# duanyiqun/DiffusionDepth

Measured on NVIDIA H100. Metric: depth maps/sec @ KITTI 352x1216, Swin-L, 20 DDIM steps, higher is better.
Workload: dtype f32 (fp32-grade products on wgmma: 3-pass fp16 split, fp32 accumulate)

## Files before the change

### diffusiondepth_b200/_cabi.py

```python
import ctypes as C
import os

_HERE = os.path.dirname(os.path.abspath(__file__))
_LIB = None


class EngineError(RuntimeError):
    """Raised for any non-zero status coming back across the C ABI."""


class DDConfig(C.Structure):
    _fields_ = [("abi_version", C.c_int32), ("variant", C.c_int32), ("batch", C.c_int32),
                ("latent_h", C.c_int32), ("latent_w", C.c_int32), ("cond_h", C.c_int32),
                ("cond_w", C.c_int32), ("num_inference_steps", C.c_int32), ("device", C.c_int32),
                ("flags", C.c_int32)]


class DDProducerConfig(C.Structure):
    _fields_ = [("num_levels", C.c_int32), ("channels", C.c_int32 * 4), ("heights", C.c_int32 * 4),
                ("widths", C.c_int32 * 4), ("has_neck", C.c_int32)]


class DDBackboneConfig(C.Structure):
    _fields_ = [("kind", C.c_int32), ("embed_dims", C.c_int32), ("depths", C.c_int32 * 4),
# ... 42 lines not shown
    "dd_denoiser_backward": (C.c_int, [C.c_void_p, C.c_void_p, C.c_void_p, C.POINTER(C.c_int64), C.c_void_p,
                                       C.c_void_p, C.c_void_p, C.POINTER(C.c_void_p), C.c_void_p, C.c_size_t,
                                       C.c_void_p]),
    "dd_denoiser_relu_inputs": (C.c_int, [C.c_void_p, C.c_void_p, C.c_void_p, C.POINTER(C.c_int64),
                                          C.POINTER(C.c_void_p), C.c_void_p, C.c_size_t, C.c_void_p]),
    "dd_denoise_backward": (C.c_int, [C.c_void_p, C.c_void_p, C.c_void_p, C.c_void_p, C.c_void_p, C.c_void_p,
                                      C.c_void_p, C.POINTER(C.c_void_p), C.POINTER(C.c_void_p), C.c_void_p,
                                      C.c_void_p, C.c_size_t, C.c_void_p]),
    "dd_decode": (C.c_int, [C.c_void_p, C.c_void_p, C.c_void_p, C.c_void_p, C.c_void_p, C.c_size_t, C.c_void_p]),
    "dd_decode_backward": (C.c_int, [C.c_void_p, C.c_void_p, C.c_void_p, C.c_void_p, C.POINTER(C.c_void_p),
                                     C.c_void_p, C.c_size_t, C.c_void_p]),
    "dd_encode": (C.c_int, [C.c_void_p, C.c_void_p, C.c_int32, C.c_int32, C.c_void_p, C.c_void_p]),
    "dd_set_codec_mode": (C.c_int, [C.c_void_p, C.c_int32]),
    "dd_codec_batch_stats": (C.c_int, [C.c_void_p, C.c_void_p, C.c_int32, C.POINTER(C.c_int32), C.c_void_p]),
    "dd_set_producer_mode": (C.c_int, [C.c_void_p, C.c_int32]),
    "dd_producer_batch_stats": (C.c_int, [C.c_void_p, C.c_void_p, C.c_int64, C.POINTER(C.c_int32), C.c_void_p]),
    "dd_producer_bn_info": (C.c_int, [C.c_void_p, C.c_int32, C.c_char_p, C.c_int32, C.POINTER(C.c_int32),
                                      C.POINTER(C.c_int64), C.POINTER(C.c_int32)]),
    "dd_last_launch_count": (C.c_int64, [C.c_void_p]),
    "dd_poll_status": (C.c_int, [C.c_void_p, C.c_void_p]),
    "dd_conv3x3": (C.c_int, [C.c_void_p, C.c_void_p, C.c_void_p, C.c_void_p, C.c_void_p, C.c_int32, C.c_int32,
                             C.c_int32, C.c_int32, C.c_int32, C.c_void_p, C.c_size_t, C.c_void_p]),
    "dd_conv3x3_workspace_bytes": (C.c_size_t, [C.c_int32, C.c_int32, C.c_int32, C.c_int32, C.c_int32]),
    "dd_conv3x3_wgrad": (C.c_int, [C.c_void_p, C.c_void_p, C.c_void_p, C.c_void_p, C.c_void_p, C.c_int32, C.c_int32,
                                   C.c_int32, C.c_int32, C.c_int32, C.c_void_p, C.c_size_t, C.c_void_p]),
    "dd_conv3x3_wgrad_workspace_bytes": (C.c_size_t, [C.c_int32, C.c_int32, C.c_int32, C.c_int32, C.c_int32]),
    "dd_gen_layer": (C.c_int, [C.c_void_p, C.POINTER(DDGenLayerDesc), C.c_void_p, C.c_void_p, C.c_void_p, C.c_void_p,
                               C.POINTER(C.c_void_p), C.c_void_p, C.c_void_p, C.c_void_p, C.c_void_p,
                               C.POINTER(C.c_int32), C.c_void_p]),
    "dd_window_attention": (C.c_int, [C.c_void_p, C.c_void_p, C.c_void_p, C.c_void_p, C.c_void_p, C.c_int32,
                                      C.c_int32, C.c_int32, C.c_int32, C.c_int32, C.c_int32, C.POINTER(C.c_int32),
                                      C.c_void_p]),
    "dd_factor_attention": (C.c_int, [C.c_void_p, C.c_void_p, C.POINTER(C.c_void_p), C.POINTER(C.c_void_p), C.c_void_p,
                                      C.c_int32, C.c_int32, C.c_int32, C.c_int32, C.POINTER(C.c_int32), C.c_void_p]),
    "dd_depthwise_conv": (C.c_int, [C.c_void_p, C.c_void_p, C.c_void_p, C.c_void_p, C.POINTER(C.c_void_p), C.c_void_p,
                                    C.c_void_p, C.c_void_p, C.c_int32, C.c_int32, C.c_int32, C.c_int32, C.c_int32,
                                    C.c_int32, C.c_int32, C.POINTER(C.c_int32), C.c_void_p]),
    "dd_layer_norm": (C.c_int, [C.c_void_p, C.c_void_p, C.c_void_p, C.c_void_p, C.c_void_p, C.c_int32, C.c_int32,
                                C.c_float, C.c_void_p]),
    "dd_bench_gemm": (C.c_int, [C.c_void_p, C.c_int32, C.c_int32, C.c_int32, C.c_int32, C.c_int32, C.POINTER(C.c_float)]),
    "dd_bench_conv": (C.c_int, [C.c_void_p, C.c_int32, C.c_int32, C.c_int32, C.POINTER(C.c_float), C.c_void_p,
                                C.c_size_t, C.c_void_p]),
    "dd_bench_pred_fold": (C.c_int, [C.c_void_p, C.c_int32, C.POINTER(C.c_float), C.c_void_p, C.c_size_t,
                                     C.c_void_p]),
}

# ... 32 lines not shown
```

### diffusiondepth_b200/csrc/conv_halo.cuh

```cuda
#pragma once
#include "conv_common.cuh"

namespace dd {

constexpr int HALO_TH = 16;
constexpr int HALO_TW = 8;

template <int CIN, int COUT, int BK>
struct HaloCfg {
  static_assert(BK == 16 || BK == 32, "bad K chunk");
  static_assert((CIN % BK == 0 || CIN < BK) && CIN % 16 == 0, "bad K chunk");
  static constexpr int KC = (CIN + BK - 1) / BK;
  static constexpr int KSTEPS = (CIN < BK ? CIN : BK) / 16;
  static constexpr int ROW_BYTES = BK * 2;
  static constexpr int STRIP_ROWS = (HALO_TH + 2) * HALO_TW;
  static constexpr int STRIP_BYTES = STRIP_ROWS * ROW_BYTES;
  static constexpr int STRIP_PAD = (STRIP_BYTES + 1023) / 1024 * 1024;
  static constexpr int DX_STRIDE = 2 * STRIP_PAD;
  static constexpr int A_SLOT = 3 * DX_STRIDE;
  static constexpr int A_SLOTS = 2;
  static constexpr int B_TILE = COUT * ROW_BYTES;
  static constexpr int B_TILE_PAD = (B_TILE + 1023) / 1024 * 1024;
  static constexpr int B_SLOT = 2 * B_TILE_PAD;
  static constexpr int NWG = COUT > 128 ? 2 : 1;
  static constexpr int NW = COUT / NWG;
  static constexpr int THREADS = 128 * (1 + NWG);
  static constexpr int CH = NWG > 1 ? 16 : (NW < 32 ? NW : 32);
  static constexpr int LD = CH + 1;
  static constexpr int STAGE_BYTES = NWG * 128 * LD * 4;
  static constexpr int CTRL_BYTES = 1024;
  static constexpr int BUDGET = 227 * 1024 - 1024 - CTRL_BYTES - STAGE_BYTES - A_SLOTS * A_SLOT;
  static constexpr int B_SLOTS_RAW = BUDGET / B_SLOT;
  static constexpr bool B_RESIDENT = (9 * KC * B_SLOT <= 40 * 1024) && (9 * KC <= B_SLOTS_RAW);
  static constexpr int B_SLOTS = B_RESIDENT ? 9 * KC : (B_SLOTS_RAW > 8 ? 8 : B_SLOTS_RAW);
  static_assert(B_SLOTS >= 2, "B ring too small");
  static_assert(NWG == 1 || B_SLOTS >= 3, "256-wide layers: the producer must be able to run two taps ahead");
  static constexpr int SMEM_BYTES = A_SLOTS * A_SLOT + B_SLOTS * B_SLOT + 1024 + CTRL_BYTES + STAGE_BYTES;
  static_assert(SMEM_BYTES <= 232448, "exceeds the 227 KB dynamic shared memory limit");
  static constexpr int A_TX = 6 * STRIP_BYTES;
  static constexpr int B_TX = 2 * B_TILE;
  static constexpr int GROUP_CH = COUT / 4;
  static constexpr int GPW = NW >= GROUP_CH ? NW / GROUP_CH : 1;
  static_assert(NW % GROUP_CH == 0, "a warpgroup's columns cover whole GroupNorm groups");
};

template <int CIN, int COUT, int BK, int EPI>
__global__ void __launch_bounds__((HaloCfg<CIN, COUT, BK>::THREADS), 1)
conv3x3_halo_kernel(const __grid_constant__ CUtensorMap tmA_hi, const __grid_constant__ CUtensorMap tmA_lo,
                    const __grid_constant__ CUtensorMap tmB_hi, const __grid_constant__ CUtensorMap tmB_lo,
                    const ConvArgs p) {
  using C = HaloCfg<CIN, COUT, BK>;
  constexpr int NW = C::NW;
  extern __shared__ uint8_t smem_raw[];
  uint8_t* smem = reinterpret_cast<uint8_t*>((reinterpret_cast<uintptr_t>(smem_raw) + 1023) & ~uintptr_t(1023));
  uint8_t* a_ring = smem;
  uint8_t* b_ring = smem + C::A_SLOTS * C::A_SLOT;
  uint8_t* ctrl = b_ring + C::B_SLOTS * C::B_SLOT;
  uint64_t* a_full = reinterpret_cast<uint64_t*>(ctrl);
  uint64_t* a_empty = a_full + C::A_SLOTS;
  uint64_t* b_full = a_empty + C::A_SLOTS;
  uint64_t* b_empty = b_full + C::B_SLOTS;
  float* red = reinterpret_cast<float*>(b_empty + C::B_SLOTS);
  float* stage = reinterpret_cast<float*>(ctrl + C::CTRL_BYTES);

  const int warp = threadIdx.x >> 5;
  const int lane = threadIdx.x & 31;

  if (threadIdx.x == 0) {
    tma_prefetch_desc(&tmA_hi);
    tma_prefetch_desc(&tmA_lo);
    tma_prefetch_desc(&tmB_hi);
    tma_prefetch_desc(&tmB_lo);
    for (int s = 0; s < C::A_SLOTS; ++s) {
      mbar_init(&a_full[s], 1);
      mbar_init(&a_empty[s], C::NWG);
    }
    for (int s = 0; s < C::B_SLOTS; ++s) {
      mbar_init(&b_full[s], 1);
      mbar_init(&b_empty[s], C::NWG);
    }
    fence_barrier_init();
  }
  __syncthreads();

  if (warp < 4) {
    if constexpr (C::NWG > 1) setmaxnreg_dec<40>();
    if (warp == 0) {
      const bool leader = elect_one();
      int sa = 0;
      uint32_t pa = 0;
      for (int tile = blockIdx.x; tile < p.num_tiles; tile += gridDim.x) {
        const int tx = tile % p.tiles_x, ty = (tile / p.tiles_x) % p.tiles_y, img = tile / (p.tiles_x * p.tiles_y);
        const int x0 = tx * HALO_TW, y0 = ty * HALO_TH;
        for (int kc = 0; kc < C::KC; ++kc) {
          mbar_wait(&a_empty[sa], pa ^ 1);
          uint8_t* s = a_ring + sa * C::A_SLOT;
          if (leader) {
            mbar_arrive_expect_tx(&a_full[sa], C::A_TX);
#pragma unroll
            for (int dx = 0; dx < 3; ++dx) {
              tma_load_4d(s + (2 * dx) * C::STRIP_PAD, &tmA_hi, &a_full[sa], kc * BK, x0 + dx - 1, y0 - 1, img);
              tma_load_4d(s + (2 * dx + 1) * C::STRIP_PAD, &tmA_lo, &a_full[sa], kc * BK, x0 + dx - 1, y0 - 1, img);
            }
          }
          __syncwarp();
          if (++sa == C::A_SLOTS) {
            sa = 0;
            pa ^= 1;
          }
        }
      }
    } else if (warp == 1) {
      const bool leader = elect_one();
      int sb = 0;
      uint32_t pb = 0;
      for (int tile = blockIdx.x; tile < p.num_tiles; tile += gridDim.x) {
        if (C::B_RESIDENT && tile != static_cast<int>(blockIdx.x)) break;
        for (int kc = 0; kc < C::KC; ++kc) {
          for (int tap = 0; tap < 9; ++tap) {
            mbar_wait(&b_empty[sb], pb ^ 1);
            uint8_t* s = b_ring + sb * C::B_SLOT;
            if (leader) {
              mbar_arrive_expect_tx(&b_full[sb], C::B_TX);
              tma_load_3d(s, &tmB_hi, &b_full[sb], kc * BK, 0, tap);
              tma_load_3d(s + C::B_TILE_PAD, &tmB_lo, &b_full[sb], kc * BK, 0, tap);
            }
            __syncwarp();
            if (++sb == C::B_SLOTS) {
              sb = 0;
              pb ^= 1;
            }
          }
        }
      }
    }
  } else {
    if constexpr (C::NWG > 1) setmaxnreg_inc<232>();
    const int wg = (warp >> 2) - 1;
    const int t = threadIdx.x & 127;
    const int q = t >> 5;
    const bool signal = (t == 0);
    float* S = stage + wg * 128 * C::LD;
    const int m = t;
    const int r = m >> 3, c = m & 7;
    const uint32_t b_off = static_cast<uint32_t>(wg * NW);
    int sa = 0, sb = 0, par = 0;
    uint32_t pa = 0, pb = 0;
    float acc[2][NW / 2];

    for (int tile = blockIdx.x; tile < p.num_tiles; tile += gridDim.x) {
      int prev_b = -1, prev_a = -1;
      auto retire_prev = [&]() {
        mbar_arrive_if(&b_empty[prev_b < 0 ? 0 : prev_b], signal && prev_b >= 0);
        mbar_arrive_if(&a_empty[prev_a < 0 ? 0 : prev_a], signal && prev_a >= 0);
        prev_b = prev_a = -1;
      };
      {
        for (int kc = 0; kc < C::KC; ++kc) {
          mbar_wait(&a_full[sa], pa);
          const uint32_t a_base = smem_u32(a_ring + sa * C::A_SLOT);
          for (int tap = 0; tap < 9; ++tap) {
            const int dy = tap / 3, dx = tap % 3;
            mbar_wait(&b_full[sb], C::B_RESIDENT ? 0u : pb);
            const uint32_t sa_hi = a_base + dx * C::DX_STRIDE + dy * HALO_TW * C::ROW_BYTES;
            const uint32_t sa_lo = sa_hi + C::STRIP_PAD;
            const uint32_t sb_hi = smem_u32(b_ring + sb * C::B_SLOT) + b_off * C::ROW_BYTES;
            const uint32_t sb_lo = sb_hi + C::B_TILE_PAD;
            wgmma_fence();
#pragma unroll
            for (int h = 0; h < 2; ++h) {
              const uint32_t ho = static_cast<uint32_t>(h * 64 * C::ROW_BYTES);
#pragma unroll
              for (int k = 0; k < C::KSTEPS; ++k) {
                const uint64_t a_hi = wgmma_desc(sa_hi + ho + k * 32, C::ROW_BYTES);
                const uint64_t a_lo = wgmma_desc(sa_lo + ho + k * 32, C::ROW_BYTES);
                const uint64_t b_hi = wgmma_desc(sb_hi + k * 32, C::ROW_BYTES);
                const uint64_t b_lo = wgmma_desc(sb_lo + k * 32, C::ROW_BYTES);
                wgmma_f16<NW>(acc[h], a_lo, b_hi, (kc | tap | k) != 0 ? 1u : 0u);
                wgmma_f16<NW>(acc[h], a_hi, b_lo, 1u);
                wgmma_f16<NW>(acc[h], a_hi, b_hi, 1u);
              }
            }
            wgmma_commit();
            wgmma_wait<1>();
            retire_prev();
            if (!C::B_RESIDENT) prev_b = sb;
            if (tap == 8) prev_a = sa;
            if (++sb == C::B_SLOTS) {
              sb = 0;
              pb ^= 1;
            }
          }
          if (++sa == C::A_SLOTS) {
            sa = 0;
            pa ^= 1;
          }
        }
      }
      wgmma_wait<0>();
      wgmma_fence_regs(acc[0]);
      wgmma_fence_regs(acc[1]);
      retire_prev();

      const int tx = tile % p.tiles_x, ty = (tile / p.tiles_x) % p.tiles_y, img = tile / (p.tiles_x * p.tiles_y);
      const int x = tx * HALO_TW + c, y = ty * HALO_TH + r;
      const bool valid = (x < p.W) && (y < p.H);
      const size_t pix = (static_cast<size_t>(img) * p.H + y) * p.W + x;
      const uint32_t vmask = __ballot_sync(0xffffffffu, valid);
      const uint32_t row_off = static_cast<uint32_t>(pix * COUT);
      float tsum[C::GPW], tsq[C::GPW];
#pragma unroll
      for (int g = 0; g < C::GPW; ++g) tsum[g] = tsq[g] = 0.f;
      bool overflow = false;
#pragma unroll
      for (int cj = 0; cj < NW / C::CH; ++cj) {
        const int ch0 = wg * NW + cj * C::CH;
        named_bar_sync(2 + wg, 128);
        stage_acc_cols<NW, C::CH, C::LD>(acc[0], S, 0, cj * C::CH / 8);
        stage_acc_cols<NW, C::CH, C::LD>(acc[1], S, 64, cj * C::CH / 8);
        named_bar_sync(2 + wg, 128);
        float v[C::CH];
#pragma unroll
        for (int j = 0; j < C::CH; ++j) v[j] = fmaf(S[m * C::LD + j], p.acc_scale, __ldg(p.bias + ch0 + j));
        if constexpr (EPI == EPI_F32_STATS) {
          if (valid) {
#pragma unroll
            for (int j = 0; j < C::CH; ++j) {
              const int g = (cj * C::CH + j) / C::GROUP_CH;
              tsum[g] += v[j];
              tsq[g] = fmaf(v[j], v[j], tsq[g]);
            }
          }
        }
        if constexpr (EPI == EPI_F32_STATS || EPI == EPI_F32) {
#pragma unroll
          for (int j = 0; j < C::CH; ++j) S[m * C::LD + j] = v[j];
          __syncwarp();
          if constexpr (C::CH == 32) {
#pragma unroll 8
// ... 14 lines not shown
        } else if (valid) {
          {
            __align__(16) __half hi[C::CH];
            __align__(16) __half lo[C::CH];
#pragma unroll
            for (int j = 0; j < C::CH; ++j) {
              const float s = v[j] * p.split_scale;
              overflow |= (fabsf(s) > 60000.f);
              hi[j] = __float2half_rn(s);
              lo[j] = __float2half_rn(s - __half2float(hi[j]));
            }
            uint4* dh = reinterpret_cast<uint4*>(p.out_hi + pix * COUT + ch0);
            uint4* dl = reinterpret_cast<uint4*>(p.out_lo + pix * COUT + ch0);
#pragma unroll
            for (int j = 0; j < C::CH / 8; ++j) {
              dh[j] = reinterpret_cast<const uint4*>(hi)[j];
              dl[j] = reinterpret_cast<const uint4*>(lo)[j];
            }
          }
        }
      }

      if constexpr (EPI == EPI_F32_STATS) {
        const int cw = wg * 4 + q;
#pragma unroll
        for (int g = 0; g < 4; ++g) {
          const int gl = g - (C::NWG > 1 ? wg * C::GPW : 0);
          float s = 0.f, s2 = 0.f;
#pragma unroll
          for (int k = 0; k < C::GPW; ++k)
            if (k == gl) {
              s = tsum[k];
              s2 = tsq[k];
            }
#pragma unroll
          for (int o = 16; o > 0; o >>= 1) {
            s += __shfl_xor_sync(0xffffffffu, s, o);
            s2 += __shfl_xor_sync(0xffffffffu, s2, o);
          }
          if (lane == 0) {
            red[((par * 4 * C::NWG + cw) * 4 + g) * 2 + 0] = s;
            red[((par * 4 * C::NWG + cw) * 4 + g) * 2 + 1] = s2;
          }
        }
        named_bar_sync(1, 128 * C::NWG);
        const int e = threadIdx.x - 128;
        if (e < 8) {
          const int g = e >> 1, which = e & 1;
          float tt = 0.f;
#pragma unroll
          for (int w = 0; w < 4 * C::NWG; ++w) tt += red[((par * 4 * C::NWG + w) * 4 + g) * 2 + which];
          p.stats_partial[(static_cast<size_t>(tile) * 4 + g) * 2 + which] = tt;
        }
        par ^= 1;
      }
      if constexpr (EPI == EPI_SPLIT) {
        if (overflow) atomicOr(p.status, 1);
      }
    }
  }
}

}
```

### diffusiondepth_b200/csrc/engine.cu

```cuda
#include <cuda.h>
#include <cuda_runtime.h>
#include <math.h>
#include <stdio.h>
#include <stdlib.h>
#include <string.h>

#include <algorithm>
#include <map>
#include <string>
#include <vector>

#include "../../include/dd_engine.h"
#include "kernels.cuh"
#include "convgen.cuh"
#include "conv_halo.cuh"
#include "pred_fold.cuh"
#include "swin.cuh"
#include "mpvit.cuh"
#include "backward.cuh"
#include "codec_train.cuh"
#include "producer_train.cuh"

namespace {

// ... 1074 lines not shown

int dev_alloc(std::vector<void*>& owned, void** p, size_t bytes) {
  cudaError_t err = cudaMalloc(p, bytes);
  if (err != cudaSuccess) return fail(DD_ERR_CUDA, std::string("cudaMalloc: ") + cudaGetErrorString(err));
  owned.push_back(*p);
  return DD_OK;
}
int dev_alloc(dd_engine* e, void** p, size_t bytes) { return dev_alloc(e->owned, p, bytes); }

template <typename T>
int dev_array(dd_engine* e, T** p, size_t elems) {
  return dev_alloc(e->owned, reinterpret_cast<void**>(p), elems * sizeof(T));
}

int alloc_layer(dd_engine* e, ConvLayer& L, int cout, int cin) {
  L.sid = shape_id(cin, cout);
  if (L.sid < 0) return fail(DD_ERR_UNSUPPORTED, "unsupported conv shape");
  const size_t n = static_cast<size_t>(cout) * cin * 9;
  int rc;
  if ((rc = dev_array(e, &L.w_hi, n))) return rc;
  if ((rc = dev_array(e, &L.w_lo, n))) return rc;
  if ((rc = dev_array(e, &L.w_simt, n))) return rc;
  if ((rc = dev_array(e, &L.bias, cout))) return rc;
  if ((rc = make_weight_map(&L.mh_hi, L.w_hi, cout, cin, 9, kHaloBK[L.sid], cout))) return rc;
  return make_weight_map(&L.mh_lo, L.w_lo, cout, cin, 9, kHaloBK[L.sid], cout);
}

constexpr float kProdScale = 16.f;

void bn_fold_host(const float* const* bn, int ch, float* scale, float* shift) {
  for (int c = 0; c < ch; ++c) {
    const double sc = static_cast<double>(bn[0][c]) / sqrt(static_cast<double>(bn[3][c]) + 1e-5);
    scale[c] = static_cast<float>(sc);
    shift[c] = static_cast<float>(static_cast<double>(bn[1][c]) - static_cast<double>(bn[2][c]) * sc);
  }
}
int bn_fold(const float* const* bn, int ch, std::vector<float>& scale, std::vector<float>& shift, cudaStream_t st) {
  std::vector<float> v[4];
  for (int i = 0; i < 4; ++i) {
    v[i].resize(ch);
    CUDA_TRY(cudaMemcpyAsync(v[i].data(), bn[i], ch * 4, cudaMemcpyDeviceToHost, st));
  }
  CUDA_TRY(cudaStreamSynchronize(st));
  scale.resize(ch);
  shift.resize(ch);
  const float* host[4] = {v[0].data(), v[1].data(), v[2].data(), v[3].data()};
  bn_fold_host(host, ch, scale.data(), shift.data());
  return DD_OK;
// ... 2137 lines not shown
  a.H = height;
  a.W = width;
  a.h = h->cfg.latent_h;
  a.w = h->cfg.latent_w;
  dim3 grid((a.w + 15) / 16, (a.h + 15) / 16, h->cfg.batch);
  dd::encoder_kernel<<<grid, 256, 0, st>>>(a);
  return check_launch("encoder");
}

int64_t dd_last_launch_count(dd_handle h) { return h ? h->launches : 0; }

int dd_poll_status(dd_handle h, void* cuda_stream) {
  if (!h) return fail(DD_ERR_INVALID, "null handle");
  if (!h->status) return DD_OK;
  CUDA_TRY(cudaSetDevice(h->cfg.device));
  return poll_status(h, static_cast<cudaStream_t>(cuda_stream));
}

size_t dd_conv3x3_workspace_bytes(int32_t batch, int32_t cin, int32_t cout, int32_t height, int32_t width) {
  Conv3x3Ws v;
  return conv3x3_layout(nullptr, batch, cin, cout, height, width, v);
}

int dd_conv3x3(dd_handle h, const float* x, const float* w, const float* b, float* y, int32_t batch, int32_t cin,
               int32_t cout, int32_t height, int32_t width, void* workspace, size_t workspace_bytes, void* cuda_stream) {
  if (!h || !x || !w || !b || !y) return fail(DD_ERR_INVALID, "null argument");
  const int sid = shape_id(cin, cout);
  if (sid < 0) return fail(DD_ERR_UNSUPPORTED, "conv shape not on the DiffusionDepth hot path");
  if (workspace_bytes < dd_conv3x3_workspace_bytes(batch, cin, cout, height, width) ||
      (reinterpret_cast<uintptr_t>(workspace) & 1023))
    return fail(DD_ERR_INVALID, "conv workspace too small or misaligned");
  cudaStream_t st = static_cast<cudaStream_t>(cuda_stream);
  CUDA_TRY(cudaSetDevice(h->cfg.device));
  const size_t BP = static_cast<size_t>(batch) * height * width;
  const size_t nw = static_cast<size_t>(cin) * cout * 9;
  Conv3x3Ws v;
  conv3x3_layout(workspace, batch, cin, cout, height, width, v);
  CUDA_TRY(cudaMemsetAsync(v.status, 0, 64, st));
  int rc;
  if ((rc = transpose_in(x, v.xn, batch, cin, height * width, st))) return rc;
  float* amax_dev = reinterpret_cast<float*>(v.status) + 8;
  float sx, sw;
  if ((rc = split_scale_of(v.xn, std::min<size_t>(BP * cin, 1u << 30), amax_dev, st, &sx))) return rc;
  if ((rc = split_scale_of(w, nw, amax_dev, st, &sw))) return rc;
  dd::split_planes_kernel<<<132 * 8, 256, 0, st>>>(v.xn, v.x.hi, v.x.lo, BP * cin / 4, sx, v.status);
  if ((rc = check_launch("split_planes"))) return rc;
  dd::pack_conv_weight_kernel<<<128, 256, 0, st>>>(w, v.w.hi, v.w.lo, v.wsimt, cout, cin, sw);
  if ((rc = check_launch("pack_conv_weight"))) return rc;
  dd::ConvArgs a;
  a.B = batch;
  a.H = height;
  a.W = width;
  a.bias = b;
  a.acc_scale = 1.f / (sx * sw);
  a.y32 = v.yn;
  a.stats_partial = nullptr;
  a.out_hi = nullptr;
  a.out_lo = nullptr;
  a.out_a8 = a.out_l8 = nullptr;
  a.split_scale = 1.f;
  a.status = v.status;
  const bool simt = (h->cfg.flags & DD_FLAG_SIMT_CONV) != 0;
  CUtensorMap mb_hi{}, mb_lo{};
  if (!simt) {
    if ((rc = make_weight_map(&mb_hi, v.w.hi, cout, cin, 9, kHaloBK[sid], cout))) return rc;
    if ((rc = make_weight_map(&mb_lo, v.w.lo, cout, cin, 9, kHaloBK[sid], cout))) return rc;
  }
  if ((rc = launch_conv3x3(sid, dd::EPI_F32, simt, a, v.x.hi, v.x.lo, sx, v.wsimt, mb_hi, mb_lo, h->sm_count, st)))
    return rc;
  if ((rc = check_launch("conv3x3"))) return rc;
  return transpose_out(v.yn, y, batch, cout, height * width, st);
}

size_t dd_conv3x3_wgrad_workspace_bytes(int32_t batch, int32_t cin, int32_t cout, int32_t height, int32_t width) {
  WgradWs v;
  return wgrad_layout(nullptr, batch, cin, cout, height, width, v);
}

int dd_conv3x3_wgrad(dd_handle h, const float* x, const float* dy, float* dw, float* db, int32_t batch, int32_t cin,
                     int32_t cout, int32_t height, int32_t width, void* workspace, size_t workspace_bytes,
                     void* cuda_stream) {
  if (!h || !x || !dy || !dw || !db) return fail(DD_ERR_INVALID, "null argument");
  if (shape_id(cin, cout) < 0) return fail(DD_ERR_UNSUPPORTED, "conv shape not on the DiffusionDepth hot path");
  if (batch < 1 || height < 1 || width < 1) return fail(DD_ERR_INVALID, "empty geometry");
  if (workspace_bytes < dd_conv3x3_wgrad_workspace_bytes(batch, cin, cout, height, width) ||
      (reinterpret_cast<uintptr_t>(workspace) & 1023))
    return fail(DD_ERR_INVALID, "wgrad workspace too small or misaligned");
  cudaStream_t st = static_cast<cudaStream_t>(cuda_stream);
  CUDA_TRY(cudaSetDevice(h->cfg.device));
  const int P = height * width;
  const size_t BP = static_cast<size_t>(batch) * P;
  WgradWs v;
  wgrad_layout(workspace, batch, cin, cout, height, width, v);
  float* scratch = reinterpret_cast<float*>(v.status) + 8;
// ... 240 lines not shown
```

### diffusiondepth_b200/engine.py

```python
import ctypes as C
from typing import Dict, Optional, Sequence, Tuple

import torch

from . import _cabi
from ._cabi import EngineError

DENOISER_KEYS = (
    "model.noise_embedding.0.weight", "model.noise_embedding.0.bias", "model.noise_embedding.1.weight",
    "model.noise_embedding.1.bias", "model.noise_embedding.3.weight", "model.noise_embedding.3.bias",
    "model.noise_embedding.4.weight", "model.noise_embedding.4.bias", "model.time_embedding.weight",
    "model.pred.0.weight", "model.pred.0.bias", "model.pred.1.weight", "model.pred.1.bias",
    "model.pred.3.weight", "model.pred.3.bias", "model.pred.4.weight", "model.pred.4.bias")
FUSE_KEYS = ("model.upsample_fuse.convA.conv.weight", "model.upsample_fuse.convA.conv.bias",
             "model.upsample_fuse.convB.conv.weight", "model.upsample_fuse.convB.conv.bias")
ENCODER_KEYS = (
    "depth_transform.conv_transform.0.0.weight", "depth_transform.conv_transform.0.1.weight",
    "depth_transform.conv_transform.0.1.bias", "depth_transform.conv_transform.0.1.running_mean",
    "depth_transform.conv_transform.0.1.running_var", "depth_transform.conv_transform.1.0.weight",
    "depth_transform.conv_transform.1.1.weight", "depth_transform.conv_transform.1.1.bias",
    "depth_transform.conv_transform.1.1.running_mean", "depth_transform.conv_transform.1.1.running_var")
_PARAM_SHAPES = {
    "model.noise_embedding.0.weight": (64, 16, 3, 3), "model.noise_embedding.0.bias": (64,),
    "model.noise_embedding.1.weight": (64,), "model.noise_embedding.1.bias": (64,),
# ... 60 lines not shown
class DenoiseEngine:

    def __init__(self, variant: str, batch: int, latent_hw: Sequence[int], cond_hw: Sequence[int],
                 num_inference_steps: int, device: torch.device, cuda_graph: bool = True,
                 simt_conv: bool = False, check_range: bool = False, halo_conv: bool = True,
                 swap_narrow: bool = True, pair_wide: bool = True, step_decode: bool = False, workspace_pool=None,
                 fp8_corr: bool = True, backward: bool = False, loop_backward: bool = False,
                 chain_pred: bool = False, producer_train: bool = False):
        self.lib = _cabi.load_library()
        device = torch.device(device)
        if device.type != "cuda":
            raise EngineError("DenoiseEngine runs on CUDA (sm_90a) only; there is no CPU path")
        self.device = device
        self.variant = variant
        self.batch, self.latent_hw, self.cond_hw = int(batch), tuple(latent_hw), tuple(cond_hw)
        self.steps = int(num_inference_steps)
        flags = (_cabi.FLAG_CUDA_GRAPH if cuda_graph else 0) | (_cabi.FLAG_SIMT_CONV if simt_conv else 0) | \
                (_cabi.FLAG_CHECK_RANGE if check_range else 0) | (_cabi.FLAG_HALO_CONV if halo_conv else 0) | \
                (_cabi.FLAG_SWAP_NARROW if swap_narrow else 0) | (_cabi.FLAG_PAIR_WIDE if pair_wide else 0) | \
                (_cabi.FLAG_STEP_DECODE if step_decode else 0) | (_cabi.FLAG_FP8_CORR if fp8_corr else 0) | \
                (_cabi.FLAG_BACKWARD if backward else 0) | (_cabi.FLAG_LOOP_BACKWARD if loop_backward else 0) | \
                (_cabi.FLAG_CHAIN_PRED if chain_pred else 0) | (_cabi.FLAG_PRODUCER_TRAIN if producer_train else 0)
        self.producer_train = bool(producer_train)
        self.fp8_corr = bool(fp8_corr)
        self.backward = bool(backward or loop_backward)
        self.loop_backward = bool(loop_backward)
        self.step_decode = bool(step_decode)
        cfg = _cabi.DDConfig(_cabi.ABI_VERSION, {"res": _cabi.VARIANT_RES, "swin": _cabi.VARIANT_SWIN}[variant],
                             self.batch, self.latent_hw[0], self.latent_hw[1], self.cond_hw[0], self.cond_hw[1],
                             self.steps, device.index if device.index is not None else torch.cuda.current_device(),
                             flags)
        h = C.c_void_p()
        _cabi.check(self.lib.dd_create(C.byref(cfg), C.byref(h)))
        self._h = h
        self._ws: Optional[torch.Tensor] = None
        self._pool = workspace_pool
        self._keep = []
        self.producers = None
        self.backbone = None

    def load_weights(self, tensors: Dict[str, torch.Tensor]):
        keys = DENOISER_KEYS + DECODER_KEYS + (FUSE_KEYS if self.variant == "swin" else ())
        if all(k in tensors for k in ENCODER_KEYS):
            keys = keys + ENCODER_KEYS
        if self.backbone is not None:
            keys = keys + tuple(k for k in tensors if k.startswith("backbone.") and tensors[k].is_floating_point())
# ... 264 lines not shown
        rec = torch.empty(total, device=self.device, dtype=torch.float32)
        n = C.c_int32()
        _cabi.check(self.lib.dd_producer_batch_stats(self._h, _ptr(rec), total, C.byref(n), C.c_void_p(self._stream())))
        return {k: (rec[o:o + c], rec[o + c:o + 2 * c]) for k, c, o, f in info if f}

    def decode(self, latent: torch.Tensor, want_logits=False):
        B, (h, w) = self.batch, self.latent_hw
        self._check_in(latent, (B, 16, h, w))
        depth = torch.empty(B, 1, 2 * h, 2 * w, device=self.device, dtype=torch.float32)
        logits = torch.empty_like(depth) if want_logits else None
        _cabi.check(self.lib.dd_decode(self._h, _ptr(latent), _ptr(logits), _ptr(depth), *self._ws_args()))
        return depth, logits

    def conv3x3(self, x: torch.Tensor, w: torch.Tensor, b: torch.Tensor) -> torch.Tensor:
        B, cin, H, W = x.shape
        cout = w.shape[0]
        x, w, b = (_f32(t, self.device) for t in (x, w, b))
        y = torch.empty(B, cout, H, W, device=self.device, dtype=torch.float32)
        need = int(self.lib.dd_conv3x3_workspace_bytes(B, cin, cout, H, W))
        ws = torch.empty(need + 1024, dtype=torch.uint8, device=self.device)
        _cabi.check(self.lib.dd_conv3x3(self._h, _ptr(x), _ptr(w), _ptr(b), _ptr(y), B, cin, cout, H, W,
                                        C.c_void_p(self._aligned(ws)), need, C.c_void_p(self._stream())))
        return y

    def conv3x3_wgrad(self, x: torch.Tensor, dy: torch.Tensor):
        B, cin, H, W = x.shape
        cout = dy.shape[1]
        if tuple(dy.shape) != (B, cout, H, W):
            raise EngineError(f"dy {tuple(dy.shape)} does not match x {tuple(x.shape)}")
        x, dy = _f32(x, self.device), _f32(dy, self.device)
        dw = torch.empty(cout, cin, 3, 3, device=self.device, dtype=torch.float32)
        db = torch.empty(cout, device=self.device, dtype=torch.float32)
        need = int(self.lib.dd_conv3x3_wgrad_workspace_bytes(B, cin, cout, H, W))
        ws = torch.empty(need + 1024, dtype=torch.uint8, device=self.device)
        _cabi.check(self.lib.dd_conv3x3_wgrad(self._h, _ptr(x), _ptr(dy), _ptr(dw), _ptr(db), B, cin, cout, H, W,
                                              C.c_void_p(self._aligned(ws)), need, C.c_void_p(self._stream())))
        return dw, db

    def gen_layer(self, x0: torch.Tensor, w: torch.Tensor, x1: Optional[torch.Tensor] = None,
                  bias: Optional[torch.Tensor] = None, bn=None, add: Optional[torch.Tensor] = None,
                  stride: int = 1, transposed: bool = False, act: int = 0, add_first: bool = False, cin: int = 0,
                  ld_out: int = 0, ch_off: int = 0, n_tile: int = 0, alt_tile: int = 0, y32=True, planes=None):
        dev = self.device
        x0, x1, w, bias, add = (_f32(t, dev) for t in (x0, x1, w, bias, add))
        bn = None if bn is None else [_f32(t, dev) for t in bn]
        d = _cabi.DDGenLayerDesc()
# ... 104 lines not shown
```

### include/dd_engine.h

```cpp
#ifndef DD_ENGINE_H_
#define DD_ENGINE_H_

#include <stddef.h>
#include <stdint.h>

#ifdef __cplusplus
extern "C" {
#endif

#define DD_ABI_VERSION 1

typedef struct dd_engine* dd_handle;

enum dd_status {
  DD_OK = 0,
  DD_ERR_INVALID = 1,
  DD_ERR_CUDA = 2,
  DD_ERR_UNSUPPORTED = 3,
  DD_ERR_RANGE = 4
};

enum dd_variant {
  DD_VARIANT_RES = 0,
  DD_VARIANT_SWIN = 1
// ... 109 lines not shown
int dd_encode(dd_handle h, const float* depth, int32_t height, int32_t width, float* latent_out, void* cuda_stream);

enum dd_codec_mode { DD_CODEC_EVAL = 0, DD_CODEC_TRAIN = 1 };
int dd_set_codec_mode(dd_handle h, int32_t mode);

int dd_codec_batch_stats(dd_handle h, float* dev_out, int32_t capacity, int32_t* n_out, void* cuda_stream);

enum dd_producer_mode { DD_PRODUCER_EVAL = 0, DD_PRODUCER_TRAIN = 1 };
int dd_set_producer_mode(dd_handle h, int32_t mode);

int dd_producer_batch_stats(dd_handle h, float* dev_out, int64_t capacity, int32_t* n_out, void* cuda_stream);

int dd_producer_bn_info(dd_handle h, int32_t i, char* key, int32_t key_capacity, int32_t* channels, int64_t* offset,
                        int32_t* fresh);

int dd_poll_status(dd_handle h, void* cuda_stream);

int64_t dd_last_launch_count(dd_handle h);

int dd_conv3x3(dd_handle h, const float* x, const float* w, const float* b, float* y, int32_t batch, int32_t cin,
               int32_t cout, int32_t height, int32_t width, void* workspace, size_t workspace_bytes,
               void* cuda_stream);
size_t dd_conv3x3_workspace_bytes(int32_t batch, int32_t cin, int32_t cout, int32_t height, int32_t width);

int dd_conv3x3_wgrad(dd_handle h, const float* x, const float* dy, float* dw, float* db, int32_t batch, int32_t cin,
                     int32_t cout, int32_t height, int32_t width, void* workspace, size_t workspace_bytes,
                     void* cuda_stream);
size_t dd_conv3x3_wgrad_workspace_bytes(int32_t batch, int32_t cin, int32_t cout, int32_t height, int32_t width);

typedef struct dd_gen_layer_desc {
  int32_t taps;
  int32_t stride;
  int32_t transposed;
  int32_t act;
  int32_t add_first;
  int32_t tokens;
  int32_t batch, height, width;
  int32_t src_h, src_w;
  int32_t c0, c1;
  int32_t cin;
  int32_t cout;
  int32_t ld_out, ch_off;
  int32_t n_tile;
  int32_t alt_tile;
} dd_gen_layer_desc;

// ... 32 lines not shown
```

Baseline: 27.81.

## Ping-pong two consumer warpgroups over column units in halo conv kernel

The halo 3x3 conv kernel now splits output channels into units, at most 128 columns each, and alternates them between two consumer warpgroups. Named barriers hand the MMA phase back and forth, so one warpgroup's epilogue overlaps the other's wgmma mainloop. It replaces the old scheme where both warpgroups split the columns of the same tile. Weight maps load per-unit column slices, the A ring gains a third slot when weights are resident, and GroupNorm stats are reduced per unit. A standalone conv3x3_epi API is added for testing epilogues. The cost is that each unit reloads the A tiles, the ring-index arithmetic is more complex, and narrow layers now always run two consumer warpgroups.

```diff
diff --git a/diffusiondepth_b200/_cabi.py b/diffusiondepth_b200/_cabi.py
--- a/diffusiondepth_b200/_cabi.py
+++ b/diffusiondepth_b200/_cabi.py
@@ -88,6 +88,9 @@
     "dd_conv3x3": (C.c_int, [C.c_void_p, C.c_void_p, C.c_void_p, C.c_void_p, C.c_void_p, C.c_int32, C.c_int32,
                              C.c_int32, C.c_int32, C.c_int32, C.c_void_p, C.c_size_t, C.c_void_p]),
     "dd_conv3x3_workspace_bytes": (C.c_size_t, [C.c_int32, C.c_int32, C.c_int32, C.c_int32, C.c_int32]),
+    "dd_conv3x3_epi": (C.c_int, [C.c_void_p, C.c_void_p, C.c_void_p, C.c_void_p, C.c_int32, C.c_void_p, C.c_void_p,
+                                 C.c_void_p, C.c_void_p, C.c_float, C.c_int32, C.c_int32, C.c_int32, C.c_int32,
+                                 C.c_int32, C.c_void_p, C.c_size_t, C.c_void_p]),
     "dd_conv3x3_wgrad": (C.c_int, [C.c_void_p, C.c_void_p, C.c_void_p, C.c_void_p, C.c_void_p, C.c_int32, C.c_int32,
                                    C.c_int32, C.c_int32, C.c_int32, C.c_void_p, C.c_size_t, C.c_void_p]),
     "dd_conv3x3_wgrad_workspace_bytes": (C.c_size_t, [C.c_int32, C.c_int32, C.c_int32, C.c_int32, C.c_int32]),
diff --git a/diffusiondepth_b200/csrc/conv_halo.cuh b/diffusiondepth_b200/csrc/conv_halo.cuh
--- a/diffusiondepth_b200/csrc/conv_halo.cuh
+++ b/diffusiondepth_b200/csrc/conv_halo.cuh
@@ -5,6 +5,8 @@
 
 constexpr int HALO_TH = 16;
 constexpr int HALO_TW = 8;
+
+constexpr int halo_unit_cols(int cout) { return cout > 128 ? cout / 2 : cout; }
 
 template <int CIN, int COUT, int BK>
 struct HaloCfg {
@@ -18,30 +20,31 @@
   static constexpr int STRIP_PAD = (STRIP_BYTES + 1023) / 1024 * 1024;
   static constexpr int DX_STRIDE = 2 * STRIP_PAD;
   static constexpr int A_SLOT = 3 * DX_STRIDE;
-  static constexpr int A_SLOTS = 2;
-  static constexpr int B_TILE = COUT * ROW_BYTES;
+  static constexpr int NW = halo_unit_cols(COUT);
+  static constexpr int UNITS = COUT / NW;
+  static constexpr int THREADS = 384;
+  static constexpr int B_TILE = NW * ROW_BYTES;
   static constexpr int B_TILE_PAD = (B_TILE + 1023) / 1024 * 1024;
   static constexpr int B_SLOT = 2 * B_TILE_PAD;
-  static constexpr int NWG = COUT > 128 ? 2 : 1;
-  static constexpr int NW = COUT / NWG;
-  static constexpr int THREADS = 128 * (1 + NWG);
-  static constexpr int CH = NWG > 1 ? 16 : (NW < 32 ? NW : 32);
+  static constexpr bool B_RESIDENT = 9 * KC * B_SLOT <= 40 * 1024;
+  static constexpr int A_SLOTS = B_RESIDENT ? 3 : 2;
+  static constexpr int CH = NW == 128 ? 16 : (NW < 32 ? NW : 32);
   static constexpr int LD = CH + 1;
-  static constexpr int STAGE_BYTES = NWG * 128 * LD * 4;
+  static constexpr int STAGE_BYTES = 2 * 128 * LD * 4;
   static constexpr int CTRL_BYTES = 1024;
   static constexpr int BUDGET = 227 * 1024 - 1024 - CTRL_BYTES - STAGE_BYTES - A_SLOTS * A_SLOT;
   static constexpr int B_SLOTS_RAW = BUDGET / B_SLOT;
-  static constexpr bool B_RESIDENT = (9 * KC * B_SLOT <= 40 * 1024) && (9 * KC <= B_SLOTS_RAW);
   static constexpr int B_SLOTS = B_RESIDENT ? 9 * KC : (B_SLOTS_RAW > 8 ? 8 : B_SLOTS_RAW);
-  static_assert(B_SLOTS >= 2, "B ring too small");
-  static_assert(NWG == 1 || B_SLOTS >= 3, "256-wide layers: the producer must be able to run two taps ahead");
+  static_assert(!B_RESIDENT || 9 * KC <= B_SLOTS_RAW, "resident weights do not fit");
+  static_assert(B_RESIDENT || B_SLOTS >= 6, "the weight producer must be able to run five taps ahead of the MMAs");
+  static_assert(8 * (2 * A_SLOTS + 2 * B_SLOTS) + 2 * 2 * 4 * 4 * 2 * 4 <= CTRL_BYTES, "control block overflows");
   static constexpr int SMEM_BYTES = A_SLOTS * A_SLOT + B_SLOTS * B_SLOT + 1024 + CTRL_BYTES + STAGE_BYTES;
   static_assert(SMEM_BYTES <= 232448, "exceeds the 227 KB dynamic shared memory limit");
   static constexpr int A_TX = 6 * STRIP_BYTES;
   static constexpr int B_TX = 2 * B_TILE;
   static constexpr int GROUP_CH = COUT / 4;
-  static constexpr int GPW = NW >= GROUP_CH ? NW / GROUP_CH : 1;
-  static_assert(NW % GROUP_CH == 0, "a warpgroup's columns cover whole GroupNorm groups");
+  static constexpr int GPW = NW / GROUP_CH;
+  static_assert(NW % GROUP_CH == 0, "a unit's columns cover whole GroupNorm groups");
 };
 
 template <int CIN, int COUT, int BK, int EPI>
@@ -73,18 +76,18 @@
     tma_prefetch_desc(&tmB_lo);
     for (int s = 0; s < C::A_SLOTS; ++s) {
       mbar_init(&a_full[s], 1);
-      mbar_init(&a_empty[s], C::NWG);
+      mbar_init(&a_empty[s], 1);
     }
     for (int s = 0; s < C::B_SLOTS; ++s) {
       mbar_init(&b_full[s], 1);
-      mbar_init(&b_empty[s], C::NWG);
+      mbar_init(&b_empty[s], 1);
     }
     fence_barrier_init();
   }
   __syncthreads();
 
   if (warp < 4) {
-    if constexpr (C::NWG > 1) setmaxnreg_dec<40>();
+    setmaxnreg_dec<40>();
     if (warp == 0) {
       const bool leader = elect_one();
       int sa = 0;
@@ -92,21 +95,23 @@
       for (int tile = blockIdx.x; tile < p.num_tiles; tile += gridDim.x) {
         const int tx = tile % p.tiles_x, ty = (tile / p.tiles_x) % p.tiles_y, img = tile / (p.tiles_x * p.tiles_y);
         const int x0 = tx * HALO_TW, y0 = ty * HALO_TH;
-        for (int kc = 0; kc < C::KC; ++kc) {
-          mbar_wait(&a_empty[sa], pa ^ 1);
-          uint8_t* s = a_ring + sa * C::A_SLOT;
-          if (leader) {
-            mbar_arrive_expect_tx(&a_full[sa], C::A_TX);
-#pragma unroll
-            for (int dx = 0; dx < 3; ++dx) {
-              tma_load_4d(s + (2 * dx) * C::STRIP_PAD, &tmA_hi, &a_full[sa], kc * BK, x0 + dx - 1, y0 - 1, img);
-              tma_load_4d(s + (2 * dx + 1) * C::STRIP_PAD, &tmA_lo, &a_full[sa], kc * BK, x0 + dx - 1, y0 - 1, img);
-            }
-          }
-          __syncwarp();
-          if (++sa == C::A_SLOTS) {
-            sa = 0;
-            pa ^= 1;
+        for (int u = 0; u < C::UNITS; ++u) {
+          for (int kc = 0; kc < C::KC; ++kc) {
+            mbar_wait(&a_empty[sa], pa ^ 1);
+            uint8_t* s = a_ring + sa * C::A_SLOT;
+            if (leader) {
+              mbar_arrive_expect_tx(&a_full[sa], C::A_TX);
+#pragma unroll
+              for (int dx = 0; dx < 3; ++dx) {
+                tma_load_4d(s + (2 * dx) * C::STRIP_PAD, &tmA_hi, &a_full[sa], kc * BK, x0 + dx - 1, y0 - 1, img);
+                tma_load_4d(s + (2 * dx + 1) * C::STRIP_PAD, &tmA_lo, &a_full[sa], kc * BK, x0 + dx - 1, y0 - 1, img);
+              }
+            }
+            __syncwarp();
+            if (++sa == C::A_SLOTS) {
+              sa = 0;
+              pa ^= 1;
+            }
           }
         }
       }
@@ -116,39 +121,48 @@
       uint32_t pb = 0;
       for (int tile = blockIdx.x; tile < p.num_tiles; tile += gridDim.x) {
         if (C::B_RESIDENT && tile != static_cast<int>(blockIdx.x)) break;
-        for (int kc = 0; kc < C::KC; ++kc) {
-          for (int tap = 0; tap < 9; ++tap) {
-            mbar_wait(&b_empty[sb], pb ^ 1);
-            uint8_t* s = b_ring + sb * C::B_SLOT;
-            if (leader) {
-              mbar_arrive_expect_tx(&b_full[sb], C::B_TX);
-              tma_load_3d(s, &tmB_hi, &b_full[sb], kc * BK, 0, tap);
-              tma_load_3d(s + C::B_TILE_PAD, &tmB_lo, &b_full[sb], kc * BK, 0, tap);
-            }
-            __syncwarp();
-            if (++sb == C::B_SLOTS) {
-              sb = 0;
-              pb ^= 1;
+        for (int u = 0; u < C::UNITS; ++u) {
+          for (int kc = 0; kc < C::KC; ++kc) {
+            for (int tap = 0; tap < 9; ++tap) {
+              mbar_wait(&b_empty[sb], pb ^ 1);
+              uint8_t* s = b_ring + sb * C::B_SLOT;
+              if (leader) {
+                mbar_arrive_expect_tx(&b_full[sb], C::B_TX);
+                tma_load_3d(s, &tmB_hi, &b_full[sb], kc * BK, u * NW, tap);
+                tma_load_3d(s + C::B_TILE_PAD, &tmB_lo, &b_full[sb], kc * BK, u * NW, tap);
+              }
+              __syncwarp();
+              if (++sb == C::B_SLOTS) {
+                sb = 0;
+                pb ^= 1;
+              }
             }
           }
         }
       }
     }
   } else {
-    if constexpr (C::NWG > 1) setmaxnreg_inc<232>();
+    setmaxnreg_inc<232>();
     const int wg = (warp >> 2) - 1;
     const int t = threadIdx.x & 127;
     const int q = t >> 5;
     const bool signal = (t == 0);
     float* S = stage + wg * 128 * C::LD;
+    float* R = red + wg * 2 * 4 * 4 * 2;
     const int m = t;
     const int r = m >> 3, c = m & 7;
-    const uint32_t b_off = static_cast<uint32_t>(wg * NW);
-    int sa = 0, sb = 0, par = 0;
-    uint32_t pa = 0, pb = 0;
+    int par = 0;
+    int unit = -1;
     float acc[2][NW / 2];
 
     for (int tile = blockIdx.x; tile < p.num_tiles; tile += gridDim.x) {
+    for (int u = 0; u < C::UNITS; ++u) {
+      if (((++unit) & 1) != wg) continue;
+      if (unit > 0) named_bar_sync(4 + wg, 256);
+      int sa = (unit * C::KC) % C::A_SLOTS;
+      uint32_t pa = ((unit * C::KC) / C::A_SLOTS) & 1;
+      int sb = C::B_RESIDENT ? 0 : (unit * 9 * C::KC) % C::B_SLOTS;
+      uint32_t pb = C::B_RESIDENT ? 0u : ((unit * 9 * C::KC) / C::B_SLOTS) & 1;
       int prev_b = -1, prev_a = -1;
       auto retire_prev = [&]() {
         mbar_arrive_if(&b_empty[prev_b < 0 ? 0 : prev_b], signal && prev_b >= 0);
@@ -161,10 +175,10 @@
           const uint32_t a_base = smem_u32(a_ring + sa * C::A_SLOT);
           for (int tap = 0; tap < 9; ++tap) {
             const int dy = tap / 3, dx = tap % 3;
-            mbar_wait(&b_full[sb], C::B_RESIDENT ? 0u : pb);
+            mbar_wait(&b_full[sb], pb);
             const uint32_t sa_hi = a_base + dx * C::DX_STRIDE + dy * HALO_TW * C::ROW_BYTES;
             const uint32_t sa_lo = sa_hi + C::STRIP_PAD;
-            const uint32_t sb_hi = smem_u32(b_ring + sb * C::B_SLOT) + b_off * C::ROW_BYTES;
+            const uint32_t sb_hi = smem_u32(b_ring + sb * C::B_SLOT);
             const uint32_t sb_lo = sb_hi + C::B_TILE_PAD;
             wgmma_fence();
 #pragma unroll
@@ -188,7 +202,7 @@
             if (tap == 8) prev_a = sa;
             if (++sb == C::B_SLOTS) {
               sb = 0;
-              pb ^= 1;
+              pb ^= C::B_RESIDENT ? 0u : 1u;
             }
           }
           if (++sa == C::A_SLOTS) {
@@ -197,6 +211,8 @@
           }
         }
       }
+      if (u + 1 < C::UNITS || tile + static_cast<int>(gridDim.x) < p.num_tiles)
+        named_bar_arrive(4 + (wg ^ 1), 256);
       wgmma_wait<0>();
       wgmma_fence_regs(acc[0]);
       wgmma_fence_regs(acc[1]);
@@ -214,7 +230,7 @@
       bool overflow = false;
 #pragma unroll
       for (int cj = 0; cj < NW / C::CH; ++cj) {
-        const int ch0 = wg * NW + cj * C::CH;
+        const int ch0 = u * NW + cj * C::CH;
         named_bar_sync(2 + wg, 128);
         stage_acc_cols<NW, C::CH, C::LD>(acc[0], S, 0, cj * C::CH / 8);
         stage_acc_cols<NW, C::CH, C::LD>(acc[1], S, 64, cj * C::CH / 8);
@@ -275,35 +291,26 @@
       }
 
       if constexpr (EPI == EPI_F32_STATS) {
-        const int cw = wg * 4 + q;
-#pragma unroll
-        for (int g = 0; g < 4; ++g) {
-          const int gl = g - (C::NWG > 1 ? wg * C::GPW : 0);
-          float s = 0.f, s2 = 0.f;
-#pragma unroll
-          for (int k = 0; k < C::GPW; ++k)
-            if (k == gl) {
-              s = tsum[k];
-              s2 = tsq[k];
-            }
+#pragma unroll
+        for (int g = 0; g < C::GPW; ++g) {
+          float s = tsum[g], s2 = tsq[g];
 #pragma unroll
           for (int o = 16; o > 0; o >>= 1) {
             s += __shfl_xor_sync(0xffffffffu, s, o);
             s2 += __shfl_xor_sync(0xffffffffu, s2, o);
           }
           if (lane == 0) {
-            red[((par * 4 * C::NWG + cw) * 4 + g) * 2 + 0] = s;
-            red[((par * 4 * C::NWG + cw) * 4 + g) * 2 + 1] = s2;
-          }
-        }
-        named_bar_sync(1, 128 * C::NWG);
-        const int e = threadIdx.x - 128;
-        if (e < 8) {
-          const int g = e >> 1, which = e & 1;
+            R[((par * 4 + q) * 4 + g) * 2 + 0] = s;
+            R[((par * 4 + q) * 4 + g) * 2 + 1] = s2;
+          }
+        }
+        named_bar_sync(2 + wg, 128);
+        if (t < 2 * C::GPW) {
+          const int g = t >> 1, which = t & 1;
           float tt = 0.f;
 #pragma unroll
-          for (int w = 0; w < 4 * C::NWG; ++w) tt += red[((par * 4 * C::NWG + w) * 4 + g) * 2 + which];
-          p.stats_partial[(static_cast<size_t>(tile) * 4 + g) * 2 + which] = tt;
+          for (int w = 0; w < 4; ++w) tt += R[((par * 4 + w) * 4 + g) * 2 + which];
+          p.stats_partial[(static_cast<size_t>(tile) * 4 + u * C::GPW + g) * 2 + which] = tt;
         }
         par ^= 1;
       }
@@ -311,6 +318,7 @@
         if (overflow) atomicOr(p.status, 1);
       }
     }
+    }
   }
 }
 
diff --git a/diffusiondepth_b200/csrc/engine.cu b/diffusiondepth_b200/csrc/engine.cu
--- a/diffusiondepth_b200/csrc/engine.cu
+++ b/diffusiondepth_b200/csrc/engine.cu
@@ -1120,8 +1120,8 @@
   if ((rc = dev_array(e, &L.w_lo, n))) return rc;
   if ((rc = dev_array(e, &L.w_simt, n))) return rc;
   if ((rc = dev_array(e, &L.bias, cout))) return rc;
-  if ((rc = make_weight_map(&L.mh_hi, L.w_hi, cout, cin, 9, kHaloBK[L.sid], cout))) return rc;
-  return make_weight_map(&L.mh_lo, L.w_lo, cout, cin, 9, kHaloBK[L.sid], cout);
+  if ((rc = make_weight_map(&L.mh_hi, L.w_hi, cout, cin, 9, kHaloBK[L.sid], dd::halo_unit_cols(cout)))) return rc;
+  return make_weight_map(&L.mh_lo, L.w_lo, cout, cin, 9, kHaloBK[L.sid], dd::halo_unit_cols(cout));
 }
 
 constexpr float kProdScale = 16.f;
@@ -3305,19 +3305,18 @@
   return conv3x3_layout(nullptr, batch, cin, cout, height, width, v);
 }
 
-int dd_conv3x3(dd_handle h, const float* x, const float* w, const float* b, float* y, int32_t batch, int32_t cin,
-               int32_t cout, int32_t height, int32_t width, void* workspace, size_t workspace_bytes, void* cuda_stream) {
-  if (!h || !x || !w || !b || !y) return fail(DD_ERR_INVALID, "null argument");
+static int conv3x3_standalone(dd_handle h, const float* x, const float* w, const float* b, int epi, float* y32,
+                              float* stats, __half* out_hi, __half* out_lo, float split_scale, int32_t batch,
+                              int32_t cin, int32_t cout, int32_t height, int32_t width, void* workspace,
+                              size_t workspace_bytes, cudaStream_t st, Conv3x3Ws& v) {
   const int sid = shape_id(cin, cout);
   if (sid < 0) return fail(DD_ERR_UNSUPPORTED, "conv shape not on the DiffusionDepth hot path");
   if (workspace_bytes < dd_conv3x3_workspace_bytes(batch, cin, cout, height, width) ||
       (reinterpret_cast<uintptr_t>(workspace) & 1023))
     return fail(DD_ERR_INVALID, "conv workspace too small or misaligned");
-  cudaStream_t st = static_cast<cudaStream_t>(cuda_stream);
   CUDA_TRY(cudaSetDevice(h->cfg.device));
   const size_t BP = static_cast<size_t>(batch) * height * width;
   const size_t nw = static_cast<size_t>(cin) * cout * 9;
-  Conv3x3Ws v;
   conv3x3_layout(workspace, batch, cin, cout, height, width, v);
   CUDA_TRY(cudaMemsetAsync(v.status, 0, 64, st));
   int rc;
@@ -3336,23 +3335,47 @@
   a.W = width;
   a.bias = b;
   a.acc_scale = 1.f / (sx * sw);
-  a.y32 = v.yn;
-  a.stats_partial = nullptr;
-  a.out_hi = nullptr;
-  a.out_lo = nullptr;
+  a.y32 = y32 ? y32 : v.yn;
+  a.stats_partial = stats;
+  a.out_hi = out_hi;
+  a.out_lo = out_lo;
   a.out_a8 = a.out_l8 = nullptr;
-  a.split_scale = 1.f;
+  a.split_scale = split_scale;
   a.status = v.status;
   const bool simt = (h->cfg.flags & DD_FLAG_SIMT_CONV) != 0;
   CUtensorMap mb_hi{}, mb_lo{};
   if (!simt) {
-    if ((rc = make_weight_map(&mb_hi, v.w.hi, cout, cin, 9, kHaloBK[sid], cout))) return rc;
-    if ((rc = make_weight_map(&mb_lo, v.w.lo, cout, cin, 9, kHaloBK[sid], cout))) return rc;
-  }
-  if ((rc = launch_conv3x3(sid, dd::EPI_F32, simt, a, v.x.hi, v.x.lo, sx, v.wsimt, mb_hi, mb_lo, h->sm_count, st)))
+    if ((rc = make_weight_map(&mb_hi, v.w.hi, cout, cin, 9, kHaloBK[sid], dd::halo_unit_cols(cout)))) return rc;
+    if ((rc = make_weight_map(&mb_lo, v.w.lo, cout, cin, 9, kHaloBK[sid], dd::halo_unit_cols(cout)))) return rc;
+  }
+  if ((rc = launch_conv3x3(sid, epi, simt, a, v.x.hi, v.x.lo, sx, v.wsimt, mb_hi, mb_lo, h->sm_count, st))) return rc;
+  return check_launch("conv3x3");
+}
+
+int dd_conv3x3(dd_handle h, const float* x, const float* w, const float* b, float* y, int32_t batch, int32_t cin,
+               int32_t cout, int32_t height, int32_t width, void* workspace, size_t workspace_bytes, void* cuda_stream) {
+  if (!h || !x || !w || !b || !y) return fail(DD_ERR_INVALID, "null argument");
+  cudaStream_t st = static_cast<cudaStream_t>(cuda_stream);
+  Conv3x3Ws v;
+  int rc;
+  if ((rc = conv3x3_standalone(h, x, w, b, dd::EPI_F32, nullptr, nullptr, nullptr, nullptr, 1.f, batch, cin, cout,
+                               height, width, workspace, workspace_bytes, st, v)))
     return rc;
-  if ((rc = check_launch("conv3x3"))) return rc;
   return transpose_out(v.yn, y, batch, cout, height * width, st);
+}
+
+int dd_conv3x3_epi(dd_handle h, const float* x, const float* w, const float* b, int32_t epilogue, float* y,
+                   float* stats, void* out_hi, void* out_lo, float split_scale, int32_t batch, int32_t cin,
+                   int32_t cout, int32_t height, int32_t width, void* workspace, size_t workspace_bytes,
+                   void* cuda_stream) {
+  if (!h || !x || !w || !b) return fail(DD_ERR_INVALID, "null argument");
+  if (epilogue == dd::EPI_F32_STATS ? (!y || !stats) : epilogue == dd::EPI_SPLIT ? (!out_hi || !out_lo)
+                                                                                 : (epilogue != dd::EPI_F32 || !y))
+    return fail(DD_ERR_INVALID, "unknown epilogue or null output");
+  Conv3x3Ws v;
+  return conv3x3_standalone(h, x, w, b, epilogue, y, stats, static_cast<__half*>(out_hi), static_cast<__half*>(out_lo),
+                            split_scale, batch, cin, cout, height, width, workspace, workspace_bytes,
+                            static_cast<cudaStream_t>(cuda_stream), v);
 }
 
 size_t dd_conv3x3_wgrad_workspace_bytes(int32_t batch, int32_t cin, int32_t cout, int32_t height, int32_t width) {
diff --git a/diffusiondepth_b200/engine.py b/diffusiondepth_b200/engine.py
--- a/diffusiondepth_b200/engine.py
+++ b/diffusiondepth_b200/engine.py
@@ -106,6 +106,7 @@
                 (_cabi.FLAG_BACKWARD if backward else 0) | (_cabi.FLAG_LOOP_BACKWARD if loop_backward else 0) | \
                 (_cabi.FLAG_CHAIN_PRED if chain_pred else 0) | (_cabi.FLAG_PRODUCER_TRAIN if producer_train else 0)
         self.producer_train = bool(producer_train)
+        self.simt_conv = bool(simt_conv)
         self.fp8_corr = bool(fp8_corr)
         self.backward = bool(backward or loop_backward)
         self.loop_backward = bool(loop_backward)
@@ -416,6 +417,27 @@
         _cabi.check(self.lib.dd_conv3x3(self._h, _ptr(x), _ptr(w), _ptr(b), _ptr(y), B, cin, cout, H, W,
                                         C.c_void_p(self._aligned(ws)), need, C.c_void_p(self._stream())))
         return y
+
+    def conv3x3_epi(self, x: torch.Tensor, w: torch.Tensor, b: torch.Tensor, epilogue: str, split_scale: float = 1.0):
+        B, cin, H, W = x.shape
+        cout = w.shape[0]
+        x, w, b = (_f32(t, self.device) for t in (x, w, b))
+        mode = {"stats": 0, "split": 1, "f32": 2}[epilogue]
+        y = stats = hi = lo = None
+        if epilogue in ("stats", "f32"):
+            y = torch.empty(B, H, W, cout, device=self.device, dtype=torch.float32)
+        if epilogue == "stats":
+            th, tw = (8, 16) if self.simt_conv else (16, 8)
+            stats = torch.empty(B * -(-H // th) * -(-W // tw), 4, 2, device=self.device, dtype=torch.float32)
+        if epilogue == "split":
+            hi = torch.empty(B, H, W, cout, device=self.device, dtype=torch.float16)
+            lo = torch.empty_like(hi)
+        need = int(self.lib.dd_conv3x3_workspace_bytes(B, cin, cout, H, W))
+        ws = torch.empty(need + 1024, dtype=torch.uint8, device=self.device)
+        _cabi.check(self.lib.dd_conv3x3_epi(self._h, _ptr(x), _ptr(w), _ptr(b), mode, _ptr(y), _ptr(stats), _ptr(hi),
+                                            _ptr(lo), split_scale, B, cin, cout, H, W, C.c_void_p(self._aligned(ws)),
+                                            need, C.c_void_p(self._stream())))
+        return {"stats": (y, stats), "split": (hi, lo), "f32": y}[epilogue]
 
     def conv3x3_wgrad(self, x: torch.Tensor, dy: torch.Tensor):
         B, cin, H, W = x.shape
diff --git a/include/dd_engine.h b/include/dd_engine.h
--- a/include/dd_engine.h
+++ b/include/dd_engine.h
@@ -155,6 +155,11 @@
                int32_t cout, int32_t height, int32_t width, void* workspace, size_t workspace_bytes,
                void* cuda_stream);
 size_t dd_conv3x3_workspace_bytes(int32_t batch, int32_t cin, int32_t cout, int32_t height, int32_t width);
+
+int dd_conv3x3_epi(dd_handle h, const float* x, const float* w, const float* b, int32_t epilogue, float* y,
+                   float* stats, void* out_hi, void* out_lo, float split_scale, int32_t batch, int32_t cin,
+                   int32_t cout, int32_t height, int32_t width, void* workspace, size_t workspace_bytes,
+                   void* cuda_stream);
 
 int dd_conv3x3_wgrad(dd_handle h, const float* x, const float* dy, float* dw, float* db, int32_t batch, int32_t cin,
                      int32_t cout, int32_t height, int32_t width, void* workspace, size_t workspace_bytes,
```

Result: faster. 28.27, median of 6 (+1.7%).
